# NVIDIA/flownet2-pytorch

Hardware: AMD Instinct MI355X
Metric: image-pairs/sec, FlowNet2 custom-layer hot path (Correlation + Resample2d + ChannelNorm) fwd+bwd @ 384x512 bs8 -- the whole FlowNet2C network's fwd+bwd image-pairs/sec is flownet2c.fwd_bwd_image_pairs_per_s; corr-layer HBM GB/s vs roofline is `roofline` (higher is better)
Workload: dtype f32; 1 GPU; FlowNet2 custom-layer hot path fwd+bwd, bs8 @384x512: Correlation 8x256x48x64 (20,1,20,1,2) [BASELINE configs[1]] + Resample2d 8x3x384x512 + ChannelNorm 8x3x384x512

## Files before the change

### flownet2-pytorch_amd/csrc/correlation_f16x2_bwd.hip

```cpp
#include <type_traits>

#include "corr_params.h"
#include "f16x2_split.h"

namespace fn2 {
namespace hb {
using f16s::exp_stat;
using f16s::scale_exp;
using f16s::split2;
using f16s::to_sgpr;
using f16s::wave_sum;

typedef float f4 __attribute__((ext_vector_type(4)));
typedef float f2 __attribute__((ext_vector_type(2)));
typedef _Float16 h2 __attribute__((ext_vector_type(2)));
typedef _Float16 h8 __attribute__((ext_vector_type(8)));
typedef short s8 __attribute__((ext_vector_type(8)));
typedef unsigned u4 __attribute__((ext_vector_type(4)));
typedef unsigned u2 __attribute__((ext_vector_type(2)));
#define FN2_LDS(T) __attribute__((address_space(3))) T

#ifdef FN2_ABL_BWDTEMPORAL
constexpr int BWD_STORE_AUX = 0;
#else
constexpr int BWD_STORE_AUX = 2;
#endif
#ifdef FN2_ABL_GNT
constexpr int G_LOAD_AUX = 2;
#else
constexpr int G_LOAD_AUX = 0;
#endif
constexpr int DR = 10, D = 21, NU = 6;
constexpr int CG = 64, NCT = CG / 16;
constexpr int CK = 32;
constexpr int CHS = 288, PARS = CK * CHS, XTERM = 2 * PARS, XBUF = 2 * XTERM;
template <int FLIP> struct GL {
    static constexpr int BI = 256;
    static constexpr int TI = FLIP ? 1024 + 4 : 1024 + 32;
    static constexpr int AI = FLIP ? D * TI + 76 : D * TI + 128;
    static constexpr int IMG = 3 * AI + D * TI;
};
static_assert(GL<0>::TI % 256 == 32 && GL<0>::AI % 256 == 32 && GL<1>::TI % 128 == 4 && GL<1>::AI % 128 == 32, "gather bank pattern");
constexpr int GIMG = GL<0>::IMG;
static_assert(GL<1>::IMG <= GIMG && GIMG % 16 == 0, "G image");
constexpr int X_OFS = GIMG, ZERO_OFS = X_OFS + 2 * XBUF, LDS_BYTES = ZERO_OFS + 64;
constexpr int E_BYTES = CG * 4 * 64 * 4;
static_assert(E_BYTES <= 2 * XBUF && LDS_BYTES <= 163840, "LDS budget");

struct Args {
    const float *nbr[2];
    const float *gout;
    float *gin[2];
    int B, C, H, W;
    int NRG, NCGR;
    int nflip, flip0;
    float fC, rC;
    unsigned long long *dbg;
};

__host__ __device__ constexpr int a_blk(int role, int ab) { return role == 0 ? (ab ? 3 : 0) : role == 1 ? (ab ? 2 : 1) : role == 2 ? (ab ? 7 : 4) : (ab ? 6 : 5); }
__host__ __device__ constexpr bool meets(int a, int j) { return 2 * j + 1 >= a - 3 && 2 * j <= a + 3; }
__host__ __device__ constexpr int frag_idx(int role, int ab, int j)
{
    int idx = 0;
    for (int b = 0; b < 2; ++b)
        for (int jj = 0; jj < 4; ++jj) {
            if (b == ab && jj == j) return meets(a_blk(role, ab), j) ? idx : -1;
            if (meets(a_blk(role, b), jj)) ++idx;
        }
    return -1;
}
__host__ __device__ constexpr int frag_sub(int role, int ab, int j)
{
    int idx = 0;
    for (int jj = 0; jj < 4; ++jj) {
        if (jj == j) return meets(a_blk(role, ab), j) ? idx : -1;
        if (meets(a_blk(role, ab), jj)) ++idx;
    }
    return -1;
}
constexpr int NF = 6;
static_assert(frag_idx(0, 1, 3) == 5 && frag_idx(1, 1, 3) == -1 && frag_idx(1, 1, 2) == 5 && frag_idx(2, 1, 3) == 5 && frag_idx(3, 1, 3) == 5,
              "6 products per role");

template <int I0, int I1, class F>
__device__ __forceinline__ void static_for(F &&f)
{
    if constexpr (I0 < I1) {
        f(std::integral_constant<int, I0>{});
        static_for<I0 + 1, I1>(f);
    }
}

__device__ __forceinline__ float exact_grad(const Args &p, int flip, int n, int c, int y, int x)
{
    const long HW = (long)p.H * p.W;
    const float *X = p.nbr[flip] + ((long)n * p.C + c) * HW;
    const float *g = p.gout + (long)n * D * D * HW;
    float s = 0.0f;
    for (int tj = 0; tj < D; ++tj)
        for (int ti = 0; ti < D; ++ti) {
            const int sgn = flip ? -1 : 1;
            const int yq = y + sgn * 2 * (tj - DR), xq = x + sgn * 2 * (ti - DR);
            if (yq < 0 || yq >= p.H || xq < 0 || xq >= p.W) continue;
            const long gp = flip ? (long)yq * p.W + xq : (long)y * p.W + x;
            s = fmaf(g[(long)(tj * D + ti) * HW + gp], X[(long)yq * p.W + xq], s);
        }
    return s;
}

constexpr int NSW = 4, NWAVES = NSW + 8;
constexpr int XK = 32 / (2 * NSW);
struct XSet { u4 v[XK][2]; };

__device__ __forceinline__ int lane_now()
{
    int l;
    asm volatile("v_mbcnt_lo_u32_b32 %0, -1, 0\n\tv_mbcnt_hi_u32_b32 %0, -1, %0" : "=v"(l));
    return l;
}

template <int VAR>
__global__ __launch_bounds__(NWAVES * 64, 3) void corr_bwd_f16x2(Args p)
{
    __shared__ __attribute__((aligned(16))) char smem[LDS_BYTES];
    __shared__ int scl_k[2];
    __shared__ __attribute__((aligned(16))) float scl_sx[2][CG];

    const int tid = threadIdx.x, lane = tid & 63;
    const int wave = __builtin_amdgcn_readfirstlane(tid >> 6);
    const bool is_stage = wave < NSW;
    const int w8 = is_stage ? wave : wave - NSW;
    const int HL = p.H >> 1;
    const long HW = (long)p.H * p.W;
    const int per_fn = 2 * p.NRG * p.NCGR;
    const int ntasks = p.nflip * p.B * per_fn;
    const bool pow2 = (p.C & (p.C - 1)) == 0;
    const int lgC = pow2 ? 31 - __builtin_clz((unsigned)p.C) : 0;
    if (tid < 16) reinterpret_cast<unsigned *>(smem + ZERO_OFS)[tid] = 0u;
    unsigned long long ts[16];
#pragma unroll
    for (int i = 0; i < 16; ++i) ts[i] = 0;
    auto stamp = [&](int i) __attribute__((always_inline)) { if (VAR & 64) ts[i] = __builtin_amdgcn_s_memtime(); };
    auto dump = [&]() __attribute__((always_inline)) {
        if ((VAR & 64) && p.dbg && lane == 0 && (wave == 0 || wave == NSW)) {
            unsigned long long *d = p.dbg + (blockIdx.x * 2 + (wave ? 1 : 0)) * 16;
#pragma unroll
            for (int i = 0; i < 16; ++i) d[i] = ts[i];
        }
    };
    auto stamp_u = [&](int si, int k) __attribute__((always_inline)) {
        if (si == 0) stamp(4 + k);
        else if (si == 1) stamp(8 + k);
    };
    stamp(0);

    struct Task { int flip, n, py, rg, cg; };
    auto get_task = [&](int t) -> Task {
        Task k;
        k.cg = t % p.NCGR; t /= p.NCGR;
        k.rg = t % p.NRG; t /= p.NRG;
#ifdef FN2_ABL_FLIPOUTER
        k.py = t & 1; t >>= 1;
        k.n = t % p.B;
        k.flip = p.nflip == 2 ? t / p.B : p.flip0;
#else
        k.flip = p.nflip == 2 ? t % 2 : p.flip0;
        if (p.nflip == 2) t >>= 1;
        k.py = t & 1; t >>= 1;
        k.n = t;
#endif
        k.cg = __builtin_amdgcn_readfirstlane(k.cg); k.rg = __builtin_amdgcn_readfirstlane(k.rg);
        k.py = __builtin_amdgcn_readfirstlane(k.py); k.n = __builtin_amdgcn_readfirstlane(k.n);
        k.flip = __builtin_amdgcn_readfirstlane(k.flip);
        return k;
    };
    auto task_u = [&](const Task &k) -> URange {
        URange r = bwd_u_range(k.rg, HL, DR, NU);
#ifdef FN2_ABL_EVENU
        if (!((r.hi - r.lo) & 1)) { if (r.lo > 0) --r.lo; else ++r.hi; }
#endif
        return r;
    };

    float *Es = reinterpret_cast<float *>(smem + X_OFS);
    auto store_rows = [&](const Task &tk, int kg, int par) {
        int ln = lane_now();
        const int g = ln >> 4, xg = 4 * (ln & 15);
        constexpr int NRI = (CG + NWAVES - 1) / NWAVES;
        const int y = 2 * (4 * tk.rg + g) + tk.py;
        const bool lane_ok = 4 * tk.rg + g < HL && xg < p.W;
        const unsigned vo = lane_ok ? (unsigned)((y * p.W + xg) * 4) : 0x80000000u;
        const __amdgpu_buffer_rsrc_t rso = __builtin_amdgcn_make_buffer_rsrc(p.gin[tk.flip] + (long)tk.n * p.C * HW, 0, (unsigned)(p.C * HW * 4), 0x00020000);
        auto chan = [&](int i) { return wave + NWAVES * i; };
        auto read_row = [&](int c) {
            return *reinterpret_cast<const f4 *>(Es + (c * 4 + g) * 64 + ((xg + 8 * g + 32 * ((c >> 2) & 1)) & 63));
        };
        f4 vals[NRI];
#pragma unroll
        for (int i = 0; i < NRI; ++i) vals[i] = read_row(chan(i) & (CG - 1));
        float f = 1.0f;
        if (!pow2) asm volatile("v_mov_b32 %0, %1" : "=v"(f) : "s"(p.fC));
        const int kx_ex = -lgC;
        auto ksum_of = [&](int c) {
            const int cc = c & (CG - 1);
            const int bits = to_sgpr(__builtin_bit_cast(int, scl_sx[par][8 * (cc & 7) + (cc >> 3)]));
            return (bits >> 23) - 127 + kg;
        };
        auto scaled = [&](f4 val, int kx) {
#pragma unroll
            for (int e = 0; e < 4; ++e) val[e] = __builtin_ldexpf(val[e], kx);
            if (!pow2) { val[0] /= f; val[1] /= f; val[2] /= f; val[3] /= f; }
            return val;
        };
        unsigned bad = 0;
#pragma unroll
        for (int i = 0; i < NRI; ++i) {
            const int c = chan(i);
            if (c >= CG) continue;
#ifdef FN2_ABL_GPRESPLIT
            if (false &&
#else
            if ((VAR & 31) == 0 && lane_ok &&
#endif
                (__builtin_amdgcn_classf(vals[i][0], 0x207) | __builtin_amdgcn_classf(vals[i][1], 0x207) |
                 __builtin_amdgcn_classf(vals[i][2], 0x207) | __builtin_amdgcn_classf(vals[i][3], 0x207)))
                bad |= 1u << i;
            if (!(VAR & 4))
                __builtin_amdgcn_raw_buffer_store_b128(__builtin_bit_cast(u4, scaled(vals[i], -ksum_of(c) - lgC)), rso, (int)vo, (int)((tk.cg * CG + c) * HW * 4), BWD_STORE_AUX);
        }
        if (bad) {
#pragma unroll 1
            for (int i = 0; i < NRI; ++i) {
                if (!(bad >> i & 1)) continue;
                const int c = chan(i);
                const int ksum = ksum_of(c);
                f4 val = read_row(c);
#pragma unroll 1
                for (int e = 0; e < 4; ++e) {
                    const float cur = e == 0 ? val[0] : e == 1 ? val[1] : e == 2 ? val[2] : val[3];
                    const bool nonfin = (__builtin_bit_cast(unsigned, cur) & 0x7f800000u) == 0x7f800000u;
                    const float ex = nonfin ? exact_grad(p, tk.flip, tk.n, tk.cg * CG + c, y, xg + e) : __builtin_ldexpf(cur, -ksum);
                    val[0] = e == 0 ? ex : val[0]; val[1] = e == 1 ? ex : val[1];
                    val[2] = e == 2 ? ex : val[2]; val[3] = e == 3 ? ex : val[3];
                }
                *reinterpret_cast<f4 *>(p.gin[tk.flip] + (((long)tk.n * p.C + tk.cg * CG + c) * p.H + y) * p.W + xg) = scaled(val, kx_ex);
            }
        }
    };

    if (is_stage) {
        const int s_piece = (lane & 3) + 4 * ((lane >> 4) & 1);
        const int s_row = (lane >> 2) & 3;
        const int s_ch = 2 * w8 + (lane >> 5);
        const int s_x = 8 * s_piece;
        const int w_ofs = s_ch * CHS + (s_piece >> 1) * 64 + (s_piece & 1) * 16 + (s_row >> 1) * 32 + (s_row & 1) * 8;
        const unsigned xbytes = (unsigned)(p.C * HW * 4), gbytes = (unsigned)(D * D * HW * 4);

        auto g_dma = [&](const Task &tk, int u) {
            if (VAR & 2) return;
            const __amdgpu_buffer_rsrc_t rsg = __builtin_amdgcn_make_buffer_rsrc(const_cast<float *>(p.gout + (long)tk.n * D * D * HW), 0, gbytes, 0x00020000);
            int ln = lane_now();
            const int bi = ln >> 4, pc = ln & 15;
#pragma unroll
            for (int k = 0; k < 4 / NSW; ++k) {
                const int ai = (4 / NSW) * w8 + k;
                const int tj = tk.flip ? 20 - 4 * u - bi + ai : 4 * u + bi - ai;
                const int il = tk.flip ? 4 * tk.rg - DR + 4 * u + bi : 4 * tk.rg + ai;
                const bool ok = tj >= 0 && tj < D && il >= 0 && il < HL && 4 * pc < p.W;
                const unsigned vo = ok ? (unsigned)(((tj * D * p.H + 2 * il + tk.py) * p.W + 4 * pc) * 4) : 0x80000000u;
                const int l0 = tk.flip ? ai * GL<1>::AI : ai * GL<0>::AI, lt = tk.flip ? GL<1>::TI : GL<0>::TI;
#pragma unroll
                for (int ti = 0; ti < D; ++ti)
                    __builtin_amdgcn_raw_ptr_buffer_load_lds(rsg, (FN2_LDS(void) *)(smem + l0 + ti * lt), 16, (int)vo, ti * (int)(HW * 4), 0, G_LOAD_AUX);
            }
        };
        auto x_issue1 = [&](XSet &L, const Task &tk, int u, int ch, int k) {
            const __amdgpu_buffer_rsrc_t rsx = __builtin_amdgcn_make_buffer_rsrc(const_cast<float *>(p.nbr[tk.flip] + (long)tk.n * p.C * HW), 0, xbytes, 0x00020000);
            const int il = 4 * tk.rg - DR + 4 * u + s_row;
            const bool ok = il >= 0 && il < HL && s_x < p.W;
            const unsigned vo = ok ? (unsigned)((s_ch * HW + (long)(2 * il + tk.py) * p.W + s_x) * 4) : 0x80000000u;
            const int soff = (int)((tk.cg * CG + ch * CK + 2 * NSW * k) * HW * 4);
            if (VAR & 2) { L.v[k][0] = (u4)(0x3c000000u + lane); L.v[k][1] = L.v[k][0]; return; }
            L.v[k][0] = __builtin_amdgcn_raw_buffer_load_b128(rsx, (int)vo, soff, 0);
            L.v[k][1] = __builtin_amdgcn_raw_buffer_load_b128(rsx, (int)(vo + 16), soff, 0);
        };
        auto x_issue = [&](XSet &L, const Task &tk, int u, int ch) {
#pragma unroll
            for (int k = 0; k < XK; ++k) x_issue1(L, tk, u, ch, k);
        };
        auto x_write1 = [&](const XSet &L, char *buf, int k, float sc) {
            if (VAR & 16) { asm volatile("" ::"v"(L.v[k][0]), "v"(L.v[k][1])); return; }
#ifdef FN2_ABL_NOMUL
            const f4 x0 = __builtin_bit_cast(f4, L.v[k][0]), x1 = __builtin_bit_cast(f4, L.v[k][1]); (void)sc;
#else
            const f4 x0 = __builtin_bit_cast(f4, L.v[k][0]) * sc, x1 = __builtin_bit_cast(f4, L.v[k][1]) * sc;
#endif
            char *dst = buf + w_ofs + k * 2 * NSW * CHS;
#pragma unroll
            for (int par = 0; par < 2; ++par) {
                unsigned h01, l01, h23, l23;
                split2(x0[par], x0[2 + par], h01, l01);
                split2(x1[par], x1[2 + par], h23, l23);
                *(FN2_LDS(u2) *)(dst + par * PARS) = (u2){h01, h23};
                *(FN2_LDS(u2) *)(dst + XTERM + par * PARS) = (u2){l01, l23};
            }
            __builtin_amdgcn_sched_barrier(0);
        };
        auto dma_wait = [&]() { asm volatile("s_waitcnt vmcnt(0)" ::: "memory"); };
        constexpr int U0 = 2;
        struct Samp { u2 x, x2, g; };
        auto sample_issue = [&](const Task &tk, Samp &S) {
            int ln = lane_now();
            const __amdgpu_buffer_rsrc_t rsx = __builtin_amdgcn_make_buffer_rsrc(const_cast<float *>(p.nbr[tk.flip] + (long)tk.n * p.C * HW), 0, xbytes, 0x00020000);
            const __amdgpu_buffer_rsrc_t rsg = __builtin_amdgcn_make_buffer_rsrc(const_cast<float *>(p.gout + (long)tk.n * D * D * HW), 0, gbytes, 0x00020000);
            const int ai = ln & 3, bi = (ln >> 2) & 3, q = ln >> 4;
            const int tj = tk.flip ? 20 - 4 * U0 - bi + ai : 4 * U0 + bi - ai;
            const int ilg = tk.flip ? 4 * tk.rg - DR + 4 * U0 + bi : 4 * tk.rg + ai;
            const int x = 2 * (((((5 * ln) >> 1) & 31) * (p.W >> 1)) >> 5);
            const int c = tk.cg * CG + ln, ilx = min(4 * tk.rg + (ln & 3), HL - 1);
            const int ti = (5 * q + (ln & 3) + bi) % D;
            const unsigned ox = (ilx >= 0 && ilx < HL) ? (unsigned)((c * HW + (long)(2 * ilx + tk.py) * p.W + x) * 4) : 0x80000000u;
            const int ilx2 = min(4 * tk.rg + ((ln + 2) & 3), HL - 1), xb = (x + (p.W >> 1)) >= p.W ? x + (p.W >> 1) - p.W : x + (p.W >> 1);
            const unsigned ox2 = (ilx2 >= 0 && ilx2 < HL) ? (unsigned)((c * HW + (long)(2 * ilx2 + tk.py) * p.W + xb) * 4) : 0x80000000u;
            const unsigned og = (ilg >= 0 && ilg < HL) ? (unsigned)((((tj * D + ti) * p.H + 2 * ilg + tk.py) * p.W + x) * 4) : 0x80000000u;
#ifdef FN2_ABL_NOSAMPLELOAD
            S.x = (u2)0x3f000000u; S.x2 = S.x; S.g = (u2)0x3f000000u; (void)ox; (void)ox2; (void)og;
#else
            S.x = (VAR & 2) ? (u2)0x3f800000u : __builtin_amdgcn_raw_buffer_load_b64(rsx, (int)ox, 0, 0);
            S.x2 = (VAR & 2) ? (u2)0x3f800000u : __builtin_amdgcn_raw_buffer_load_b64(rsx, (int)ox2, 0, 0);
            S.g = (VAR & 2) ? (u2)0x3f800000u : __builtin_amdgcn_raw_buffer_load_b64(rsg, (int)og, 0, 0);
#endif
        };
        auto sample_scales = [&](const Samp &S, int &kx, int &kg) {
            const unsigned t4 = exp_stat(S.x[0]) + exp_stat(S.x[1]) + exp_stat(S.x2[0]) + exp_stat(S.x2[1]);
            const unsigned sum = t4 & 0xffffu, cnt = t4 >> 16;
            const int em = cnt ? (int)((2u * sum + cnt) / (2u * cnt)) : 0;
            const int k = f16s::T_GEO + 127 - em;
            kx = cnt == 0u ? 0 : (k < -126 ? -126 : k > 127 ? 127 : k);
            const unsigned tg = exp_stat(S.g[0]) + exp_stat(S.g[1]);
            kg = scale_exp(wave_sum(tg));
        };
        auto publish = [&](int par, int kx, int kg) {
            if (wave == 0) {
                int ln = lane_now();
                scl_sx[par][8 * (ln & 7) + (ln >> 3)] = f16s::scale_from_exp(kx);
                if (ln == 0) scl_k[1] = kg;
            }
        };
        auto pick = [](bool c, const Task &a, const Task &b) {
            Task r;
            r.flip = c ? a.flip : b.flip; r.n = c ? a.n : b.n; r.py = c ? a.py : b.py; r.rg = c ? a.rg : b.rg; r.cg = c ? a.cg : b.cg;
            return r;
        };
        XSet XA0, XA1, XB0, XB1;
        int t = (int)xcd_remap(blockIdx.x, gridDim.x);
        Samp SM;
        int kx_n = 0, kg_n = 0;
        int it = 0;
        if (t < ntasks) {
            const Task tk = get_task(t);
            const int u0 = task_u(tk).lo;
            sample_issue(tk, SM);
            x_issue(XA0, tk, u0, 0);
            x_issue(XA1, tk, u0, 1);
            g_dma(tk, u0);
            stamp(1);
            dma_wait();
            stamp(2);
            sample_scales(SM, kx_n, kg_n);
            publish(0, kx_n, kg_n);
        }
        __syncthreads();
        stamp(3);
        for (; t < ntasks; t += gridDim.x) {
            const Task tk = get_task(t);
            const bool has_next = t + (int)gridDim.x < ntasks;
            const Task tn = get_task(has_next ? t + (int)gridDim.x : t);
            const bool first = t < (int)gridDim.x;
            const int kg_cur = kg_n, par = it & 1;
            const URange ur = task_u(tk);
            const int un_lo = task_u(tn).lo;
            auto one_u = [&](int u, XSet &C0, XSet &C1, XSet &N0, XSet &N1) -> bool {
                const bool last = u == ur.hi;
                const Task t1 = pick(last, tn, tk);
                const int u1 = last ? un_lo : u + 1;
                const int si = u - ur.lo;
                const float *sxp = &scl_sx[par][8 * s_ch];
                float sc = sxp[0];
                x_issue(N0, t1, u1, 0); x_issue(N1, t1, u1, 1);
#pragma unroll
                for (int k = 0; k < 2 * XK; ++k) {
                    const float nx = sxp[k + 1 < 2 * XK ? k + 1 : k];
                    if (k < XK) x_write1(C0, smem + X_OFS, k, sc);
                    else x_write1(C1, smem + X_OFS + XBUF, k - XK, sc);
                    sc = nx;
                }
                if (first) stamp_u(si, 0);
                __syncthreads();
                if (first) stamp_u(si, 1);
                if (last && has_next) sample_issue(tn, SM);
                if (!last || has_next) g_dma(t1, u1);
                dma_wait();
                if (first) stamp_u(si, 2);
                __syncthreads();
                if (first) stamp_u(si, 3);
                return last;
            };
            for (int u = ur.lo;; u += 2) {
                if (one_u(u, XA0, XA1, XB0, XB1)) {
                    XA0 = XB0; XA1 = XB1;
                    break;
                }
                if (one_u(u + 1, XB0, XB1, XA0, XA1)) break;
            }
            if (has_next) { sample_scales(SM, kx_n, kg_n); publish(par ^ 1, kx_n, kg_n); }
            if (first) stamp(12);
            __syncthreads();
            if (first) stamp(13);
            store_rows(tk, kg_cur, par);
            __syncthreads();
            if (first) stamp(14);
            ++it;
        }
        stamp(15);
        dump();
        return;
    }

    if (VAR & 256) __builtin_amdgcn_s_setprio(2);
    const int xpar = w8 & 1;
    const int role = __builtin_amdgcn_readfirstlane(w8 >> 1);

    int itm = 0;
    int steps_run = 0;
    auto run_task = [&](const Task &tk, auto flipc, bool first) {
        constexpr int FLIP = decltype(flipc)::value;
        const int kg_cur = to_sgpr(scl_k[1]);
        const f16s::scale2_t sc_g2 = f16s::scale2_from_exp(kg_cur);
        int ln = lane_now();
        const int f_i = ln & 15, f_g = ln >> 4;
        const int f_ai = f_i >> 2, f_aj = f_i & 3;
        const int xb = xpar * PARS + f_i * CHS + f_g * 16;

        f4 acc[2][NCT];
#pragma unroll
        for (int ab = 0; ab < 2; ++ab)
#pragma unroll
            for (int ct = 0; ct < NCT; ++ct) acc[ab][ct] = (f4){0.0f, 0.0f, 0.0f, 0.0f};
        h8 gh[NF], gl[NF];

        auto gather = [&](auto role_c, auto xp_c) {
            constexpr int R = decltype(role_c)::value;
            constexpr int XP = decltype(xp_c)::value;
            typedef GL<FLIP> L;
            constexpr int SB = L::TI - 8;
            int l2 = lane_now();
            const int ai = (l2 & 15) >> 2, aj = l2 & 3, blk = (l2 >> 4) & 1, gg = l2 >> 5;
            const int lbase = FLIP ? ai * L::AI + 2 * gg * L::BI + (DR - 4 * blk + aj) * L::TI - 3 * SB + 32 * blk + 4 * XP
                                   : ai * L::AI + 2 * gg * L::BI + (DR + 4 * blk - aj) * L::TI + 8 * aj;
            const int vs = 4 * blk - aj;
            static_for<0, 2>([&](auto abc) {
                constexpr int ab = decltype(abc)::value;
                constexpr int a = a_blk(R, ab);
                static_for<0, 4>([&](auto jc) {
                    constexpr int j = decltype(jc)::value;
                    constexpr int fi = frag_idx(R, ab, j);
                    if constexpr (fi >= 0) {
                        constexpr int dj = 2 * j - a;
                        constexpr int pconst = FLIP ? -4 * dj * L::TI + 64 * j : 4 * dj * L::TI + 32 * a;
                        constexpr bool check = dj < -1 || dj + 1 > 1;
                        const int fbase = lbase + pconst;
                        f2 w[4];
                        static_for<0, 8>([&](auto sc) {
                            constexpr int s = decltype(sc)::value;
                            constexpr int bjs = s & 3, bis = s >> 2;
                            constexpr int sconst = FLIP ? bis * L::BI + (3 - bjs) * SB : bis * L::BI + bjs * L::TI;
                            const int ofs = fbase + sconst;
                            float v;
                            if (VAR & 8) v = 1.0f;
                            else if constexpr (FLIP) v = *reinterpret_cast<const float *>(smem + ofs);
#ifdef FN2_ABL_GATHER64
                            else v = (*reinterpret_cast<const f2 *>(smem + ofs))[XP];
#else
                            else v = *reinterpret_cast<const float *>(smem + ofs + 4 * XP);
#endif
                            if constexpr (check) {
                                constexpr int hi = 10 - 4 * dj - bjs, lo = -10 - 4 * dj - bjs;
                                if constexpr (hi < 4) v = vs <= hi ? v : 0.0f;
                                if constexpr (lo > -3) v = vs >= lo ? v : 0.0f;
                            }
                            w[s & 3][s >> 2] = v;
                        });
                        u4 vh, vl;
#ifdef FN2_ABL_GPRESPLIT
#pragma unroll
                        for (int q = 0; q < 4; ++q) {
                            const unsigned a0 = __builtin_bit_cast(unsigned, w[(2 * q) & 3][q >> 1]), a1 = __builtin_bit_cast(unsigned, w[(2 * q + 1) & 3][q >> 1]);
                            vh[q] = __builtin_amdgcn_perm(a1, a0, 0x05040100u);
                            vl[q] = __builtin_amdgcn_perm(a1, a0, 0x07060302u);
                        }
#else
#pragma unroll
                        for (int q = 0; q < 4; ++q) w[q] = f16s::pk_scale(w[q], sc_g2);
#pragma unroll
                        for (int q = 0; q < 4; ++q) {
                            unsigned hq, lq;
                            split2(w[(2 * q) & 3][q >> 1], w[(2 * q + 1) & 3][q >> 1], hq, lq);
                            vh[q] = hq; vl[q] = lq;
                        }
#endif
                        gh[fi] = __builtin_bit_cast(h8, vh);
                        gl[fi] = __builtin_bit_cast(h8, vl);
                        __builtin_amdgcn_sched_barrier(0);
                    }
                });
            });
        };
        auto mma = [&](auto role_c) {
            constexpr int R = decltype(role_c)::value;
            static_for<0, 4>([&](auto jc) {
                constexpr int j = decltype(jc)::value;
                constexpr int f0 = frag_idx(R, 0, j), f1 = frag_idx(R, 1, j);
                if constexpr (f0 >= 0 || f1 >= 0) {
                    static_for<0, 2>([&](auto chc) {
                        constexpr int ch = decltype(chc)::value;
                        const char *buf = smem + X_OFS + ch * XBUF;
                        h8 xh[2], xl[2];
#pragma unroll
                        for (int c2 = 0; c2 < 2; ++c2) {
                            if (VAR & 8) { xh[c2] = (h8)((_Float16)1.0f); xl[c2] = xh[c2]; }
                            else {
                                xh[c2] = *reinterpret_cast<const h8 *>(buf + xb + c2 * 16 * CHS + j * 64);
                                xl[c2] = *reinterpret_cast<const h8 *>(buf + xb + c2 * 16 * CHS + j * 64 + XTERM);
                            }
                        }
                        if (VAR & 1) {
                            asm volatile("" ::"v"(xh[0]), "v"(xl[0]), "v"(xh[1]), "v"(xl[1]));
                        } else {
                            static_for<0, 3>([&](auto prc) {
                                constexpr int pr = decltype(prc)::value;
#pragma unroll
                                for (int c2 = 0; c2 < 2; ++c2) {
                                    if constexpr (f0 >= 0)
                                        acc[0][2 * ch + c2] = __builtin_amdgcn_mfma_f32_16x16x32_f16(pr == 2 ? xl[c2] : xh[c2], pr == 1 ? gl[f0 >= 0 ? f0 : 0] : gh[f0 >= 0 ? f0 : 0], acc[0][2 * ch + c2], 0, 0, 0);
                                    if constexpr (f1 >= 0)
                                        acc[1][2 * ch + c2] = __builtin_amdgcn_mfma_f32_16x16x32_f16(pr == 2 ? xl[c2] : xh[c2], pr == 1 ? gl[f1 >= 0 ? f1 : 0] : gh[f1 >= 0 ? f1 : 0], acc[1][2 * ch + c2], 0, 0, 0);
                                }
                            });
                        }
                        __builtin_amdgcn_sched_barrier(0);
                    });
                }
            });
        };
        auto gather_x = [&](auto xp_c) {
            switch (role) {
            case 0: gather(std::integral_constant<int, 0>{}, xp_c); break;
            case 1: gather(std::integral_constant<int, 1>{}, xp_c); break;
            case 2: gather(std::integral_constant<int, 2>{}, xp_c); break;
            default: gather(std::integral_constant<int, 3>{}, xp_c); break;
            }
        };
        auto gather_d = [&]() {
            if (xpar) gather_x(std::integral_constant<int, 1>{});
            else gather_x(std::integral_constant<int, 0>{});
        };
        auto mma_d = [&]() {
            switch (role) {
            case 0: mma(std::integral_constant<int, 0>{}); break;
            case 1: mma(std::integral_constant<int, 1>{}); break;
            case 2: mma(std::integral_constant<int, 2>{}); break;
            default: mma(std::integral_constant<int, 3>{}); break;
            }
        };

        const URange ur = task_u(tk);
        const int nsteps = ur.hi - ur.lo + 1;
        for (int si = 0; si < nsteps; ++si) {
            gather_d();
            if (first) stamp_u(si, 0);
            __syncthreads();
            if (first) stamp_u(si, 1);
            mma_d();
            if (first) stamp_u(si, 2);
            __syncthreads();
            if (first) stamp_u(si, 3);
        }
        if (VAR & 64) steps_run += nsteps;
        if (first) stamp(12);

        auto scatter = [&](auto role_c) {
            constexpr int R = decltype(role_c)::value;
            static_for<0, 2>([&](auto abc) {
                constexpr int ab = decltype(abc)::value;
                constexpr int a = a_blk(R, ab);
                const int x = 8 * a + 2 * f_aj + xpar;
                static_for<0, NCT>([&](auto ctc) {
                    constexpr int ct = decltype(ctc)::value;
                    static_for<0, 4>([&](auto rc) {
                        constexpr int r = decltype(rc)::value;
                        const int c = 16 * ct + 4 * f_g + r;
                        Es[(c * 4 + f_ai) * 64 + ((x + 8 * f_ai + 32 * (f_g & 1)) & 63)] = acc[ab][ct][r];
                    });
                });
            });
        };
        switch (role) {
        case 0: scatter(std::integral_constant<int, 0>{}); break;
        case 1: scatter(std::integral_constant<int, 1>{}); break;
        case 2: scatter(std::integral_constant<int, 2>{}); break;
        default: scatter(std::integral_constant<int, 3>{}); break;
        }
        __syncthreads();
        if (first) stamp(13);
        store_rows(tk, kg_cur, itm & 1);
        __syncthreads();
        if (first) stamp(14);
    };
    __syncthreads();
    stamp(3);
    for (int t = (int)xcd_remap(blockIdx.x, gridDim.x); t < ntasks; t += gridDim.x, ++itm) {
        const Task tk = get_task(t);
        const bool first = t < (int)gridDim.x;
        if (tk.flip) run_task(tk, std::integral_constant<int, 1>{}, first);
        else run_task(tk, std::integral_constant<int, 0>{}, first);
    }
    stamp(15);
    if (VAR & 64) ts[1] = (unsigned long long)steps_run;
    dump();
}

}

bool corr_bwd_f16x2_applicable(int dtype, int C, int H, int W, int pad, int k, int md, int s1, int s2)
{
    if (dtype != FN2_F32) return false;
    if (k != 1 || s1 != 1 || s2 != 2 || pad != md || md != 2 * hb::DR) return false;
    if (C % hb::CG != 0 || C < hb::CG || (H & 1) || (W % 8) != 0) return false;
    if ((long)C * H * W * 4 >= 0x7fffffffL || (long)hb::D * hb::D * H * W * 4 >= 0x7fffffffL) return false;
    return true;
}

int corr_backward_f16x2(const float *in1, const float *in2, const float *gout, float *g1, float *g2, int B, int C, int H, int W,
                        int variant, hipStream_t s)
{
    if (!aligned(in1, 16) || !aligned(in2, 16) || !aligned(gout, 16) || !aligned(g1, 16) || !aligned(g2, 16)) return FN2_EALIGN;
    if (W > 64) return variant == 0 ? corr_backward_f16x2_wide(in1, in2, gout, g1, g2, B, C, H, W, s) : FN2_EINVAL;
    hb::Args a;
    a.nbr[0] = in2; a.nbr[1] = in1; a.gout = gout; a.gin[0] = g1; a.gin[1] = g2;
    a.B = B; a.C = C; a.H = H; a.W = W;
    a.NRG = (H / 2 + 3) / 4; a.NCGR = C / hb::CG;
    a.nflip = 2; a.flip0 = 0;
    a.fC = (float)C; a.rC = 1.0f / (float)C;
#ifdef FN2_DEBUG_BUILD
    a.dbg = (variant & 64) ? static_cast<unsigned long long *>(corr_f16x2_get_debug_buffer()) : nullptr;
#else
    a.dbg = nullptr;
#endif
    const long ntasks = 2L * B * 2 * a.NRG * a.NCGR;
    if (ntasks == 0) return FN2_OK;
    if (ntasks > 0x3fffffffL) return FN2_EINVAL;
    const unsigned grid = ntasks < 256 ? (unsigned)ntasks : 256u;
#define FN2_HB(V) case V: hipLaunchKernelGGL((hb::corr_bwd_f16x2<V>), dim3(grid), dim3(hb::NWAVES * 64), 0, s, a); return launch_status();
    switch (variant) {
        FN2_HB(0)
#ifdef FN2_DEBUG_BUILD
        FN2_HB(1) FN2_HB(2) FN2_HB(4) FN2_HB(8) FN2_HB(16) FN2_HB(6) FN2_HB(24) FN2_HB(31) FN2_HB(64) FN2_HB(256) FN2_HB(65) FN2_HB(66) FN2_HB(68) FN2_HB(72) FN2_HB(80)
#endif
    default: return FN2_EINVAL;
    }
#undef FN2_HB
}

}
```

### flownet2-pytorch_amd/csrc/f16x2_split.h

```cpp
#pragma once

namespace fn2 {
namespace f16s {

constexpr int T_GEO = -1;

__device__ __forceinline__ unsigned pk_f16(float a, float b)
{
    typedef float f2v __attribute__((ext_vector_type(2)));
    typedef _Float16 h2v __attribute__((ext_vector_type(2)));
    return __builtin_bit_cast(unsigned, __builtin_convertvector((f2v){a, b}, h2v));
}
__device__ __forceinline__ void split2(float x0, float x1, unsigned &h, unsigned &l)
{
    h = pk_f16(x0, x1);
    float r0, r1;
    asm("v_fma_mix_f32 %0, %1, -1.0, %2 op_sel_hi:[1,0,0]" : "=v"(r0) : "v"(h), "v"(x0));
    asm("v_fma_mix_f32 %0, %1, -1.0, %2 op_sel:[1,0,0] op_sel_hi:[1,0,0]" : "=v"(r1) : "v"(h), "v"(x1));
    l = pk_f16(r0, r1);
}

typedef float f2s __attribute__((ext_vector_type(2)));
typedef float f4s __attribute__((ext_vector_type(4)));
typedef unsigned long long scale2_t;
__device__ __forceinline__ f2s pk_scale(f2s v, scale2_t s2)
{
#ifdef FN2_ABL_NOMUL
    return v;
#else
    f2s r;
    asm("v_pk_mul_f32 %0, %1, %2" : "=v"(r) : "v"(v), "s"(s2));
    return r;
#endif
}
__device__ __forceinline__ f4s pk_scale4(f4s v, scale2_t s2)
{
    const f2s lo = pk_scale(__builtin_shufflevector(v, v, 0, 1), s2), hi = pk_scale(__builtin_shufflevector(v, v, 2, 3), s2);
    return __builtin_shufflevector(lo, hi, 0, 1, 2, 3);
}

__device__ __forceinline__ int to_sgpr(int v)
{
    int s;
    asm volatile("s_nop 4\n\tv_readfirstlane_b32 %0, %1\n\ts_nop 4" : "=s"(s) : "v"(v));
    return s;
}

__device__ __forceinline__ unsigned exp_stat(unsigned bits)
{
    const unsigned e = (bits >> 23) & 0xffu;
    return e + ((e != 0u ? 1u : 0u) << 16);
}
__device__ __forceinline__ unsigned wave_sum(unsigned b)
{
    b += (unsigned)__builtin_amdgcn_update_dpp(0, (int)b, 0xB1, 0xf, 0xf, false);
    b += (unsigned)__builtin_amdgcn_update_dpp(0, (int)b, 0x4E, 0xf, 0xf, false);
    b += (unsigned)__builtin_amdgcn_update_dpp(0, (int)b, 0x141, 0xf, 0xf, false);
    b += (unsigned)__builtin_amdgcn_update_dpp(0, (int)b, 0x140, 0xf, 0xf, false);
    return __builtin_amdgcn_readlane(b, 0) + __builtin_amdgcn_readlane(b, 16) + __builtin_amdgcn_readlane(b, 32) +
           __builtin_amdgcn_readlane(b, 48);
}

__device__ __forceinline__ int scale_exp(unsigned packed)
{
    const unsigned sum = packed & 0xffffu, cnt = packed >> 16;
    if (cnt == 0u) return 0;
    const int e = (int)((float)sum * __builtin_amdgcn_rcpf((float)cnt) + 0.5f);
    const int k = T_GEO + 127 - to_sgpr(e);
    return k > 127 ? 127 : k < -126 ? -126 : k;
}
__device__ __forceinline__ float scale_from_exp(int k) { return __builtin_bit_cast(float, (unsigned)(127 + k) << 23); }
__device__ __forceinline__ scale2_t scale2_from_exp(int k)
{
    const unsigned b = (unsigned)(127 + k) << 23;
    return ((scale2_t)b << 32) | b;
}

}
}
```

Baseline: 45240 image-pairs/s.

## Defer last gradient fragment split into MFMA loop to overlap VALU with matrix ops

The fp32-to-f16 hi/lo split of the last gathered gradient fragment is deferred out of the gather phase. Its scale and split pieces are interleaved between MFMA issues of the preceding pair, or run right before the first pair, so VALU work hides under matrix-core latency. Split helpers now reuse their input registers in place to cut VGPR pressure, and the role dispatch is hoisted outside the step loop. This adds scheduling fences that constrain the compiler and more complex static control flow, and the correlation backward is only one part of the measured path.

Result: no change. 45550 image-pairs/s (median of 5 runs) (+0.7%).

```diff
diff --git a/flownet2-pytorch_amd/csrc/correlation_f16x2_bwd.hip b/flownet2-pytorch_amd/csrc/correlation_f16x2_bwd.hip
--- a/flownet2-pytorch_amd/csrc/correlation_f16x2_bwd.hip
+++ b/flownet2-pytorch_amd/csrc/correlation_f16x2_bwd.hip
@@ -79,6 +79,32 @@
     }
     return -1;
 }
+__host__ __device__ constexpr int next_j(int role, int j)
+{
+    for (int jj = j + 1; jj < 4; ++jj)
+        if (meets(a_blk(role, 0), jj) || meets(a_blk(role, 1), jj)) return jj;
+    return -1;
+}
+__host__ __device__ constexpr int first_j(int role) { return next_j(role, -1); }
+__host__ __device__ constexpr int frag_ord(int role, int ab, int j)
+{
+    int n = 0;
+    for (int jj = 0; jj < 4; ++jj)
+        for (int b = 0; b < 2; ++b) {
+            if (jj == j && b == ab) return n;
+            if (meets(a_blk(role, b), jj)) ++n;
+        }
+    return n;
+}
+#ifndef FN2_BWD_NDEFER
+#ifdef FN2_ABL_EARLYSPLIT
+#define FN2_BWD_NDEFER 0
+#else
+#define FN2_BWD_NDEFER 1
+#endif
+#endif
+constexpr int NDEFER = FN2_BWD_NDEFER;
+__host__ __device__ constexpr bool deferred(int role, int ab, int j) { return frag_idx(role, ab, j) >= 0 && frag_ord(role, ab, j) >= 6 - NDEFER; }
 constexpr int NF = 6;
 static_assert(frag_idx(0, 1, 3) == 5 && frag_idx(1, 1, 3) == -1 && frag_idx(1, 1, 2) == 5 && frag_idx(2, 1, 3) == 5 && frag_idx(3, 1, 3) == 5,
               "6 products per role");
@@ -448,7 +474,33 @@
         for (int ab = 0; ab < 2; ++ab)
 #pragma unroll
             for (int ct = 0; ct < NCT; ++ct) acc[ab][ct] = (f4){0.0f, 0.0f, 0.0f, 0.0f};
-        h8 gh[NF], gl[NF];
+        f2 gw[NF][4];
+        u4 gvh[NF], gvl[NF];
+        auto split_piece = [&](auto fic, auto pc, bool fence) __attribute__((always_inline)) {
+            constexpr int fi = decltype(fic)::value, pcs = decltype(pc)::value;
+            if constexpr (pcs == 0) {
+                if (fence) asm volatile("" : "+v"(gw[fi][0]), "+v"(gw[fi][1]), "+v"(gw[fi][2]), "+v"(gw[fi][3]));
+#ifndef FN2_ABL_GPRESPLIT
+#pragma unroll
+                for (int q = 0; q < 4; ++q) f16s::pk_scale_tied(gw[fi][q], sc_g2);
+#endif
+            } else {
+                constexpr int q = pcs - 1;
+                float w0 = gw[fi][(2 * q) & 3][q >> 1], w1 = gw[fi][(2 * q + 1) & 3][q >> 1];
+#ifdef FN2_ABL_GPRESPLIT
+                const unsigned a0 = __builtin_bit_cast(unsigned, w0), a1 = __builtin_bit_cast(unsigned, w1);
+                gvh[fi][q] = __builtin_amdgcn_perm(a1, a0, 0x05040100u);
+                gvl[fi][q] = __builtin_amdgcn_perm(a1, a0, 0x07060302u);
+#else
+                unsigned hq, lq;
+                f16s::split2_tied(w0, w1, hq, lq);
+                gvh[fi][q] = hq; gvl[fi][q] = lq;
+#endif
+            }
+        };
+        auto split_all = [&](auto fic, bool fence) __attribute__((always_inline)) {
+            static_for<0, 5>([&](auto pc) { split_piece(fic, pc, fence); });
+        };
 
         auto gather = [&](auto role_c, auto xp_c) {
             constexpr int R = decltype(role_c)::value;
@@ -471,7 +523,7 @@
                         constexpr int pconst = FLIP ? -4 * dj * L::TI + 64 * j : 4 * dj * L::TI + 32 * a;
                         constexpr bool check = dj < -1 || dj + 1 > 1;
                         const int fbase = lbase + pconst;
-                        f2 w[4];
+                        f2 (&w)[4] = gw[fi];
                         static_for<0, 8>([&](auto sc) {
                             constexpr int s = decltype(sc)::value;
                             constexpr int bjs = s & 3, bis = s >> 2;
@@ -492,26 +544,8 @@
                             }
                             w[s & 3][s >> 2] = v;
                         });
-                        u4 vh, vl;
-#ifdef FN2_ABL_GPRESPLIT
-#pragma unroll
-                        for (int q = 0; q < 4; ++q) {
-                            const unsigned a0 = __builtin_bit_cast(unsigned, w[(2 * q) & 3][q >> 1]), a1 = __builtin_bit_cast(unsigned, w[(2 * q + 1) & 3][q >> 1]);
-                            vh[q] = __builtin_amdgcn_perm(a1, a0, 0x05040100u);
-                            vl[q] = __builtin_amdgcn_perm(a1, a0, 0x07060302u);
-                        }
-#else
-#pragma unroll
-                        for (int q = 0; q < 4; ++q) w[q] = f16s::pk_scale(w[q], sc_g2);
-#pragma unroll
-                        for (int q = 0; q < 4; ++q) {
-                            unsigned hq, lq;
-                            split2(w[(2 * q) & 3][q >> 1], w[(2 * q + 1) & 3][q >> 1], hq, lq);
-                            vh[q] = hq; vl[q] = lq;
-                        }
-#endif
-                        gh[fi] = __builtin_bit_cast(h8, vh);
-                        gl[fi] = __builtin_bit_cast(h8, vl);
+                        if constexpr (!deferred(R, ab, j)) split_all(std::integral_constant<int, fi>{}, false);
+                        else asm volatile("" : "+v"(w[0]), "+v"(w[1]), "+v"(w[2]), "+v"(w[3]));
                         __builtin_amdgcn_sched_barrier(0);
                     }
                 });
@@ -523,8 +557,12 @@
                 constexpr int j = decltype(jc)::value;
                 constexpr int f0 = frag_idx(R, 0, j), f1 = frag_idx(R, 1, j);
                 if constexpr (f0 >= 0 || f1 >= 0) {
+                    [[maybe_unused]] constexpr bool first_pair = j == first_j(R);
+                    constexpr int jn = next_j(R, j);
+                    constexpr int n0 = jn >= 0 && deferred(R, 0, jn) ? frag_idx(R, 0, jn) : -1, n1 = jn >= 0 && deferred(R, 1, jn) ? frag_idx(R, 1, jn) : -1;
                     static_for<0, 2>([&](auto chc) {
                         constexpr int ch = decltype(chc)::value;
+                        [[maybe_unused]] constexpr int nf = ch == 0 ? (n0 >= 0 ? n0 : n1) : (n0 >= 0 ? n1 : -1);
                         const char *buf = smem + X_OFS + ch * XBUF;
                         h8 xh[2], xl[2];
 #pragma unroll
@@ -535,57 +573,56 @@
                                 xl[c2] = *reinterpret_cast<const h8 *>(buf + xb + c2 * 16 * CHS + j * 64 + XTERM);
                             }
                         }
-                        if (VAR & 1) {
-                            asm volatile("" ::"v"(xh[0]), "v"(xl[0]), "v"(xh[1]), "v"(xl[1]));
-                        } else {
-                            static_for<0, 3>([&](auto prc) {
-                                constexpr int pr = decltype(prc)::value;
-#pragma unroll
-                                for (int c2 = 0; c2 < 2; ++c2) {
+                        if constexpr (first_pair && ch == 0 && (deferred(R, 0, j) || deferred(R, 1, j))) {
+                            __builtin_amdgcn_sched_barrier(0);
+                            if constexpr (deferred(R, 0, j)) split_all(std::integral_constant<int, f0 >= 0 ? f0 : 0>{}, true);
+                            if constexpr (deferred(R, 1, j)) split_all(std::integral_constant<int, f1 >= 0 ? f1 : 0>{}, true);
+                            __builtin_amdgcn_sched_barrier(0);
+                        }
+                        static_for<0, 3>([&](auto prc) {
+                            constexpr int pr = decltype(prc)::value;
+                            static_for<0, 2>([&](auto c2c) {
+                                constexpr int c2 = decltype(c2c)::value;
+                                if (VAR & 1) {
+                                    if (pr == 0) asm volatile("" ::"v"(xh[c2]), "v"(xl[c2]));
+                                } else {
                                     if constexpr (f0 >= 0)
-                                        acc[0][2 * ch + c2] = __builtin_amdgcn_mfma_f32_16x16x32_f16(pr == 2 ? xl[c2] : xh[c2], pr == 1 ? gl[f0 >= 0 ? f0 : 0] : gh[f0 >= 0 ? f0 : 0], acc[0][2 * ch + c2], 0, 0, 0);
+                                        acc[0][2 * ch + c2] = __builtin_amdgcn_mfma_f32_16x16x32_f16(pr == 2 ? xl[c2] : xh[c2], __builtin_bit_cast(h8, pr == 1 ? gvl[f0 >= 0 ? f0 : 0] : gvh[f0 >= 0 ? f0 : 0]), acc[0][2 * ch + c2], 0, 0, 0);
                                     if constexpr (f1 >= 0)
-                                        acc[1][2 * ch + c2] = __builtin_amdgcn_mfma_f32_16x16x32_f16(pr == 2 ? xl[c2] : xh[c2], pr == 1 ? gl[f1 >= 0 ? f1 : 0] : gh[f1 >= 0 ? f1 : 0], acc[1][2 * ch + c2], 0, 0, 0);
+                                        acc[1][2 * ch + c2] = __builtin_amdgcn_mfma_f32_16x16x32_f16(pr == 2 ? xl[c2] : xh[c2], __builtin_bit_cast(h8, pr == 1 ? gvl[f1 >= 0 ? f1 : 0] : gvh[f1 >= 0 ? f1 : 0]), acc[1][2 * ch + c2], 0, 0, 0);
+                                }
+                                constexpr int piece = 2 * pr + c2;
+                                if constexpr (nf >= 0 && piece < 5) {
+                                    split_piece(std::integral_constant<int, nf >= 0 ? nf : 0>{}, std::integral_constant<int, piece < 5 ? piece : 0>{}, true);
+                                    __builtin_amdgcn_sched_barrier(0);
                                 }
                             });
-                        }
+                        });
                         __builtin_amdgcn_sched_barrier(0);
                     });
                 }
             });
         };
-        auto gather_x = [&](auto xp_c) {
-            switch (role) {
-            case 0: gather(std::integral_constant<int, 0>{}, xp_c); break;
-            case 1: gather(std::integral_constant<int, 1>{}, xp_c); break;
-            case 2: gather(std::integral_constant<int, 2>{}, xp_c); break;
-            default: gather(std::integral_constant<int, 3>{}, xp_c); break;
-            }
-        };
-        auto gather_d = [&]() {
-            if (xpar) gather_x(std::integral_constant<int, 1>{});
-            else gather_x(std::integral_constant<int, 0>{});
-        };
-        auto mma_d = [&]() {
-            switch (role) {
-            case 0: mma(std::integral_constant<int, 0>{}); break;
-            case 1: mma(std::integral_constant<int, 1>{}); break;
-            case 2: mma(std::integral_constant<int, 2>{}); break;
-            default: mma(std::integral_constant<int, 3>{}); break;
-            }
-        };
-
         const URange ur = task_u(tk);
         const int nsteps = ur.hi - ur.lo + 1;
-        for (int si = 0; si < nsteps; ++si) {
-            gather_d();
-            if (first) stamp_u(si, 0);
-            __syncthreads();
-            if (first) stamp_u(si, 1);
-            mma_d();
-            if (first) stamp_u(si, 2);
-            __syncthreads();
-            if (first) stamp_u(si, 3);
+        auto steps = [&](auto role_c) {
+            for (int si = 0; si < nsteps; ++si) {
+                if (xpar) gather(role_c, std::integral_constant<int, 1>{});
+                else gather(role_c, std::integral_constant<int, 0>{});
+                if (first) stamp_u(si, 0);
+                __syncthreads();
+                if (first) stamp_u(si, 1);
+                mma(role_c);
+                if (first) stamp_u(si, 2);
+                __syncthreads();
+                if (first) stamp_u(si, 3);
+            }
+        };
+        switch (role) {
+        case 0: steps(std::integral_constant<int, 0>{}); break;
+        case 1: steps(std::integral_constant<int, 1>{}); break;
+        case 2: steps(std::integral_constant<int, 2>{}); break;
+        default: steps(std::integral_constant<int, 3>{}); break;
         }
         if (VAR & 64) steps_run += nsteps;
         if (first) stamp(12);
diff --git a/flownet2-pytorch_amd/csrc/f16x2_split.h b/flownet2-pytorch_amd/csrc/f16x2_split.h
--- a/flownet2-pytorch_amd/csrc/f16x2_split.h
+++ b/flownet2-pytorch_amd/csrc/f16x2_split.h
@@ -32,6 +32,19 @@
     asm("v_pk_mul_f32 %0, %1, %2" : "=v"(r) : "v"(v), "s"(s2));
     return r;
 #endif
+}
+__device__ __forceinline__ void pk_scale_tied(f2s &v, scale2_t s2)
+{
+#ifndef FN2_ABL_NOMUL
+    asm("v_pk_mul_f32 %0, %0, %1" : "+v"(v) : "s"(s2));
+#endif
+}
+__device__ __forceinline__ void split2_tied(float &x0, float &x1, unsigned &h, unsigned &l)
+{
+    h = pk_f16(x0, x1);
+    asm("v_fma_mix_f32 %0, %1, -1.0, %0 op_sel_hi:[1,0,0]" : "+v"(x0) : "v"(h));
+    asm("v_fma_mix_f32 %0, %1, -1.0, %0 op_sel:[1,0,0] op_sel_hi:[1,0,0]" : "+v"(x1) : "v"(h));
+    l = pk_f16(x0, x1);
 }
 __device__ __forceinline__ f4s pk_scale4(f4s v, scale2_t s2)
 {
```
